# TorchIO-project/torchio

Hardware: AMD Instinct MI355X
Metric: volumes/s (256^3 float32) for Compose[affine+elastic+bias+blur+noise] (higher is better)
Workload: dtype f32; 1 GPU; Compose[Affine(+-10deg,0.9-1.1,+-5mm),ElasticDeformation(7^3cp,7.5mm),BiasField,Blur(0.5-2mm),Noise] on 1x256^3 f32, per-instance params; batch_per_gpu=8, global_batch=8, noise_rng=philox, resample_precision=tight, stencil_precision=fast, parallelism=batch-split x1 (no data-path collective)

## Files before the change

torchio_amd/csrc/stencil_march.hpp:

```cpp
#pragma once

#include "common.hpp"
#include "philox_normal.hpp"

namespace tio {

constexpr int kBlock = 256;

struct ConvArgs {
  const void* src;
  void* dst;
  const void* x_orig;
  const float* taps;
  const uint8_t* skip;
  int I, J, K;
  int channels;
  int axis, radius;
  int taps_batched, tap_stride;
  int orig_dtype;
  int last_pass;
  int tiles_a;
  int bcs;
  int radius_k;
  const float* bias_coarse;
  int bias_ci, bias_cj, bias_ck;
  float bias_si, bias_sj, bias_sk;
  int noise_on, noise_batched;
  float noise_mean, noise_std;
  const float* noise_mean_b;
  const float* noise_std_b;
  uint64_t noise_seed;
  const float* noise_base;
  int fma;
};

constexpr int kMarchMaxRadius = 8;
#ifndef TIO_MARCH_AHEAD
#define TIO_MARCH_AHEAD 2
#endif
constexpr int kMarchAhead = TIO_MARCH_AHEAD;

template <int R, bool FUSE_K, bool PRE_BIAS, int POST_NOISE, bool FMA>
__global__ __launch_bounds__(kBlock, (FUSE_K && !PRE_BIAS && R <= 6) ? 4 : 1) void conv_march_kernel(const ConvArgs a) {
  constexpr int W = 2 * R + 1;
  typedef float v4f __attribute__((ext_vector_type(4)));
  typedef __attribute__((address_space(4))) const float* const_float_ptr;
  extern __shared__ __attribute__((aligned(16))) float s_mem[];
  const int lane = threadIdx.x & 63, wave = __builtin_amdgcn_readfirstlane(threadIdx.x >> 6);
  float* s_krow = s_mem + wave * 272;
  (void)s_krow;
  const int n_other = a.axis == 0 ? a.J : a.I;
  const int strip_block = a.tiles_a ? blockIdx.x : blockIdx.z;
  const int k_tile = a.tiles_a ? blockIdx.z : blockIdx.x;
  const int strip = strip_block * (kBlock / 64) + wave;
  if (strip >= n_other * a.bcs) return;
  const int other = strip % n_other;
  const int bc = strip / n_other;
  const int b = bc / a.channels;
  const int k = k_tile * 256 + 4 * lane;
  const int n = a.axis == 0 ? a.I : a.J;
  const int seg = (n + gridDim.y - 1) / gridDim.y;
  const int p_begin = blockIdx.y * seg, p_end = min(p_begin + seg, n);
  const int64_t n_spatial = static_cast<int64_t>(a.I) * a.J * a.K;
  const int64_t stride = a.axis == 0 ? static_cast<int64_t>(a.J) * a.K : a.K;
  const int64_t other_stride = a.axis == 0 ? a.K : static_cast<int64_t>(a.J) * a.K;
  const int64_t line = static_cast<int64_t>(bc) * n_spatial + other * other_stride + k;
  const float* src = static_cast<const float*>(a.src);
  float* dst = static_cast<float*>(a.dst);
  if (p_begin >= p_end || k >= a.K) return;

  if (a.skip != nullptr && a.skip[b] != 0) {
    if (a.last_pass) {
      const float* orig = static_cast<const float*>(a.x_orig);
      for (int p = p_begin; p < p_end; p++) {
        const int64_t e = line + static_cast<int64_t>(p) * stride;
        *reinterpret_cast<v4f*>(dst + e) = *reinterpret_cast<const v4f*>(orig + e);
      }
    }
    return;
  }
  const int64_t tap_base = a.taps_batched ? static_cast<int64_t>(b) * 3 * a.tap_stride : 0;
  const_float_ptr tc = (const_float_ptr)(a.taps + tap_base + static_cast<int64_t>(a.axis) * a.tap_stride);
  const_float_ptr tk = (const_float_ptr)(a.taps + tap_base + 2 * a.tap_stride);
  (void)tk;
  float tw[W];
#pragma unroll
  for (int t = 0; t < W; t++) tw[t] = tc[t];
  float tkw[17];
  (void)tkw;
  if constexpr (FUSE_K) {
    const int rk0 = a.radius_k;
#pragma unroll
    for (int jj = 0; jj < 17; jj++) {
      const int t = jj - (8 - rk0);
      tkw[jj] = (t >= 0 && t <= 2 * rk0) ? tk[t] : 0.0f;
    }
  }
  float noise_mu = a.noise_mean, noise_sd = a.noise_std;
  if constexpr (POST_NOISE != 0) {
    if (a.noise_batched) {
      noise_mu = ((const_float_ptr)a.noise_mean_b)[b];
      noise_sd = ((const_float_ptr)a.noise_std_b)[b];
    }
  }

  Lerp1D b_lk[4];
  Lerp1D b_lj{0, 0, 1.0f, 0.0f};
  float b_p0[4] = {0.f, 0.f, 0.f, 0.f}, b_p1[4] = {0.f, 0.f, 0.f, 0.f};
  int b_cur0 = -1, b_cur1 = -1;
  const float* b_fg = nullptr;
  if constexpr (PRE_BIAS) {
    b_fg = a.bias_coarse + static_cast<int64_t>(bc) * (a.bias_ci * a.bias_cj * a.bias_ck);
    b_lj = lerp_index(other, a.bias_cj, a.J, a.bias_sj);
#pragma unroll
    for (int e = 0; e < 4; e++) b_lk[e] = lerp_index(min(k + e, a.K - 1), a.bias_ck, a.K, a.bias_sk);
  }
  auto bias_row = [&](v4f v, int pos) -> v4f {
    if constexpr (PRE_BIAS) {
      const Lerp1D li = lerp_index(pos, a.bias_ci, a.I, a.bias_si);
      const int s_i = a.bias_cj * a.bias_ck, s_j = a.bias_ck;
      auto plane = [&](int ii, float (&out)[4]) {
        const float* r0 = b_fg + ii * s_i + b_lj.i0 * s_j;
        const float* r1 = b_fg + ii * s_i + b_lj.i1 * s_j;
#pragma unroll
        for (int e = 0; e < 4; e++)
          out[e] = lerp2(lerp2(r0[b_lk[e].i0], b_lk[e].l0, r0[b_lk[e].i1], b_lk[e].l1), b_lj.l0,
                         lerp2(r1[b_lk[e].i0], b_lk[e].l0, r1[b_lk[e].i1], b_lk[e].l1), b_lj.l1);
      };
      if (li.i0 != b_cur0) {
        if (li.i0 == b_cur1) {
#pragma unroll
          for (int e = 0; e < 4; e++) b_p0[e] = b_p1[e];
        } else {
          plane(li.i0, b_p0);
        }
        b_cur0 = li.i0;
      }
      if (li.i1 != b_cur1) {
        if (li.i1 == b_cur0) {
#pragma unroll
          for (int e = 0; e < 4; e++) b_p1[e] = b_p0[e];
        } else {
          plane(li.i1, b_p1);
        }
        b_cur1 = li.i1;
      }
      v.x = __fmul_rn(v.x, expf(lerp2(b_p0[0], li.l0, b_p1[0], li.l1)));
      v.y = __fmul_rn(v.y, expf(lerp2(b_p0[1], li.l0, b_p1[1], li.l1)));
      v.z = __fmul_rn(v.z, expf(lerp2(b_p0[2], li.l0, b_p1[2], li.l1)));
      v.w = __fmul_rn(v.w, expf(lerp2(b_p0[3], li.l0, b_p1[3], li.l1)));
    }
    return v;
  };
#define TIO_ROW_POS(P) min(max((P), 0), n - 1)
#define TIO_ROW_LOAD(P) (*reinterpret_cast<const v4f*>(src + line + static_cast<int64_t>(TIO_ROW_POS(P)) * stride))
  v4f win[W];
#pragma unroll
  for (int t = 0; t < 2 * R; t++) win[t] = bias_row(TIO_ROW_LOAD(p_begin - R + t), TIO_ROW_POS(p_begin - R + t));
  win[2 * R] = win[0];
  v4f nxt[kMarchAhead];
#pragma unroll
  for (int d = 0; d < kMarchAhead; d++) nxt[d] = TIO_ROW_LOAD(p_begin + R + d);
  for (int p0 = p_begin; p0 < p_end; p0 += W) {
#pragma unroll
    for (int u = 0; u < W; u++) {
      const int p = p0 + u;
      if (p >= p_end) return;
      __builtin_amdgcn_sched_barrier(0);
      win[(2 * R + u) % W] = bias_row(nxt[0], TIO_ROW_POS(p + R));
#pragma unroll
      for (int d = 0; d + 1 < kMarchAhead; d++) nxt[d] = nxt[d + 1];
      v4f zrow = {0.0f, 0.0f, 0.0f, 0.0f};
      if constexpr (POST_NOISE == 2) zrow = __builtin_nontemporal_load(reinterpret_cast<const v4f*>(a.noise_base + line + static_cast<int64_t>(p) * stride));
      (void)zrow;
      nxt[kMarchAhead - 1] = TIO_ROW_LOAD(p + R + kMarchAhead);
      float4 acc = make_float4(0.0f, 0.0f, 0.0f, 0.0f);
      if constexpr (FMA) {
#pragma unroll
        for (int t = 0; t < W; t++) {
          const v4f v = win[(u + t) % W];
          acc.x = __builtin_fmaf(tw[t], v.x, acc.x);
          acc.y = __builtin_fmaf(tw[t], v.y, acc.y);
          acc.z = __builtin_fmaf(tw[t], v.z, acc.z);
          acc.w = __builtin_fmaf(tw[t], v.w, acc.w);
        }
      } else {
#pragma unroll
        for (int t = 0; t < W; t++) {
          const v4f v = win[(u + t) % W];
          acc.x = __fadd_rn(acc.x, __fmul_rn(tw[t], v.x));
          acc.y = __fadd_rn(acc.y, __fmul_rn(tw[t], v.y));
          acc.z = __fadd_rn(acc.z, __fmul_rn(tw[t], v.z));
          acc.w = __fadd_rn(acc.w, __fmul_rn(tw[t], v.w));
        }
      }
      if constexpr (FUSE_K) {
        int rk = a.radius_k;
        if constexpr (!FMA) asm volatile("" : "+s"(rk));
        const float edge_l = __int_as_float(__builtin_amdgcn_readlane(__float_as_int(acc.x), 0));
        const float edge_r = __int_as_float(__builtin_amdgcn_readlane(__float_as_int(acc.w), a.K / 4 - 1));
        *reinterpret_cast<float4*>(s_krow + 8 + 4 * lane) = acc;
        for (int h = lane; h < 16; h += a.K / 4) {
          if (h < 8) s_krow[h] = edge_l;
          else s_krow[8 + a.K + (h - 8)] = edge_r;
        }
        __builtin_amdgcn_fence(__ATOMIC_ACQ_REL, "wavefront");
        __builtin_amdgcn_wave_barrier();
        const float4* rv = reinterpret_cast<const float4*>(s_krow + 8) + lane;
        float w[20];
#pragma unroll
        for (int d = 0; d < 5; d++) {
          const float4 c = rv[d - 2];
          w[4 * d] = c.x; w[4 * d + 1] = c.y; w[4 * d + 2] = c.z; w[4 * d + 3] = c.w;
        }
        float4 out = make_float4(0.0f, 0.0f, 0.0f, 0.0f);
        if constexpr (FMA) {
#define TIO_K_TIER(T)                                              \
  _Pragma("unroll") for (int jj = 8 - (T); jj <= 8 + (T); jj++) { \
    const float tv = tkw[jj];                                      \
    out.x = __builtin_fmaf(tv, w[jj], out.x);                      \
    out.y = __builtin_fmaf(tv, w[jj + 1], out.y);                  \
    out.z = __builtin_fmaf(tv, w[jj + 2], out.z);                  \
    out.w = __builtin_fmaf(tv, w[jj + 3], out.w);                  \
  }
          if (rk <= 4) { TIO_K_TIER(4) } else if (rk <= 6) { TIO_K_TIER(6) } else { TIO_K_TIER(8) }
#undef TIO_K_TIER
        } else {
#define TIO_K_TAP(JJ)                                       \
  {                                                         \
    const float tv = tkw[JJ];                               \
    out.x = __fadd_rn(out.x, __fmul_rn(tv, w[(JJ)]));       \
    out.y = __fadd_rn(out.y, __fmul_rn(tv, w[(JJ) + 1]));   \
    out.z = __fadd_rn(out.z, __fmul_rn(tv, w[(JJ) + 2]));   \
    out.w = __fadd_rn(out.w, __fmul_rn(tv, w[(JJ) + 3]));   \
  }
          if (rk <= 4) {
#pragma unroll
            for (int jj = 4; jj <= 12; jj++) {
              if (jj >= 7 && jj <= 9) TIO_K_TAP(jj)
              else if (jj >= 8 - rk && jj <= 8 + rk) TIO_K_TAP(jj)
            }
          } else if (rk <= 6) {
            if (rk == 6) TIO_K_TAP(2)
#pragma unroll
            for (int jj = 3; jj <= 13; jj++) TIO_K_TAP(jj)
            if (rk == 6) TIO_K_TAP(14)
          } else {
            if (rk == 8) TIO_K_TAP(0)
#pragma unroll
            for (int jj = 1; jj <= 15; jj++) TIO_K_TAP(jj)
            if (rk == 8) TIO_K_TAP(16)
          }
#undef TIO_K_TAP
        }
        acc = out;
        __builtin_amdgcn_fence(__ATOMIC_ACQ_REL, "wavefront");
        __builtin_amdgcn_wave_barrier();
        if constexpr (POST_NOISE != 0) {
          const int64_t e0 = line + static_cast<int64_t>(p) * stride;
          float z[4];
          if constexpr (POST_NOISE == 2) {
            z[0] = zrow.x; z[1] = zrow.y; z[2] = zrow.z; z[3] = zrow.w;
          } else {
            philox_normal4(a.noise_seed, 0, static_cast<uint64_t>(e0 >> 2), z);
          }
          const float mu = noise_mu, sd = noise_sd;
          acc.x = __fadd_rn(acc.x, __fadd_rn(mu, __fmul_rn(sd, z[0])));
          acc.y = __fadd_rn(acc.y, __fadd_rn(mu, __fmul_rn(sd, z[1])));
          acc.z = __fadd_rn(acc.z, __fadd_rn(mu, __fmul_rn(sd, z[2])));
          acc.w = __fadd_rn(acc.w, __fadd_rn(mu, __fmul_rn(sd, z[3])));
        }
      }
      *reinterpret_cast<float4*>(dst + line + static_cast<int64_t>(p) * stride) = acc;
    }
  }
#undef TIO_ROW_LOAD
#undef TIO_ROW_POS
}

void launch_conv_march_fused(int radius_class, int post_noise, bool fma, dim3 grid, size_t lds, hipStream_t stream, const ConvArgs& a);

}
```

Measured before the change: 6120 volumes/s.

## Specialize fused blur march kernel on runtime effective tap radius

The march body moves into an include file and is instantiated once per effective radius from 1 to R for the FMA fused-K path. At runtime each wave counts the symmetric zero outer taps in both the marching and the K filters, then dispatches to a body with a narrower register window and fewer FMAs, taking the K tier from the trimmed radius. Per-instance blur sigmas pad the tap arrays with zeros, so skipping those taps removes wasted loads and FMAs. The cost is more code size and instruction cache pressure, possible register changes from several inlined bodies, and a per-wave branch.

```diff
diff --git a/torchio_amd/csrc/stencil_march.hpp b/torchio_amd/csrc/stencil_march.hpp
--- a/torchio_amd/csrc/stencil_march.hpp
+++ b/torchio_amd/csrc/stencil_march.hpp
@@ -39,6 +39,7 @@
 #define TIO_MARCH_AHEAD 2
 #endif
 constexpr int kMarchAhead = TIO_MARCH_AHEAD;
+constexpr int kMarchOwnRadiusMax = 6;
 
 template <int R, bool FUSE_K, bool PRE_BIAS, int POST_NOISE, bool FMA>
 __global__ __launch_bounds__(kBlock, (FUSE_K && !PRE_BIAS && R <= 6) ? 4 : 1) void conv_march_kernel(const ConvArgs a) {
@@ -104,178 +105,70 @@
     }
   }
 
-  Lerp1D b_lk[4];
-  Lerp1D b_lj{0, 0, 1.0f, 0.0f};
-  float b_p0[4] = {0.f, 0.f, 0.f, 0.f}, b_p1[4] = {0.f, 0.f, 0.f, 0.f};
-  int b_cur0 = -1, b_cur1 = -1;
-  const float* b_fg = nullptr;
-  if constexpr (PRE_BIAS) {
-    b_fg = a.bias_coarse + static_cast<int64_t>(bc) * (a.bias_ci * a.bias_cj * a.bias_ck);
-    b_lj = lerp_index(other, a.bias_cj, a.J, a.bias_sj);
+  if constexpr (FMA && FUSE_K && !PRE_BIAS && R <= kMarchOwnRadiusMax) {
+    int lead = 0, lead_k = 0;
+    bool outer_zero = true;
 #pragma unroll
-    for (int e = 0; e < 4; e++) b_lk[e] = lerp_index(min(k + e, a.K - 1), a.bias_ck, a.K, a.bias_sk);
+    for (int t = 0; t < R - 1; t++) {
+      outer_zero = outer_zero && ((__float_as_int(tw[t]) | __float_as_int(tw[2 * R - t])) << 1) == 0;
+      lead += outer_zero ? 1 : 0;
+    }
+    outer_zero = true;
+#pragma unroll
+    for (int jj = 0; jj < 7; jj++) {
+      outer_zero = outer_zero && ((__float_as_int(tkw[jj]) | __float_as_int(tkw[16 - jj])) << 1) == 0;
+      lead_k += outer_zero ? 1 : 0;
+    }
+    const int r_own = R - lead;
+    int rk_tier = 8 - lead_k;
+    asm volatile("" : "+v"(rk_tier), "+v"(noise_mu), "+v"(noise_sd));
+    if (r_own == 1) {
+      constexpr int RB = 1, WB = 2 * RB + 1, tap_first = R - RB;
+#include "stencil_march_body.inc"
+      return;
+    }
+    if constexpr (R >= 2) {
+      if (r_own == 2) {
+        constexpr int RB = 2, WB = 2 * RB + 1, tap_first = R - RB;
+#include "stencil_march_body.inc"
+        return;
+      }
+    }
+    if constexpr (R >= 3) {
+      if (r_own == 3) {
+        constexpr int RB = 3, WB = 2 * RB + 1, tap_first = R - RB;
+#include "stencil_march_body.inc"
+        return;
+      }
+    }
+    if constexpr (R >= 4) {
+      if (r_own == 4) {
+        constexpr int RB = 4, WB = 2 * RB + 1, tap_first = R - RB;
+#include "stencil_march_body.inc"
+        return;
+      }
+    }
+    if constexpr (R >= 5) {
+      if (r_own == 5) {
+        constexpr int RB = 5, WB = 2 * RB + 1, tap_first = R - RB;
+#include "stencil_march_body.inc"
+        return;
+      }
+    }
+    if constexpr (R >= 6) {
+      if (r_own == 6) {
+        constexpr int RB = 6, WB = 2 * RB + 1, tap_first = R - RB;
+#include "stencil_march_body.inc"
+        return;
+      }
+    }
+    static_assert(kMarchOwnRadiusMax == 6, "one case per radius up to kMarchOwnRadiusMax");
+  } else {
+    constexpr int RB = R, WB = W, tap_first = 0;
+    const int rk_tier = a.radius_k;
+    (void)rk_tier;
+#include "stencil_march_body.inc"
   }
-  auto bias_row = [&](v4f v, int pos) -> v4f {
-    if constexpr (PRE_BIAS) {
-      const Lerp1D li = lerp_index(pos, a.bias_ci, a.I, a.bias_si);
-      const int s_i = a.bias_cj * a.bias_ck, s_j = a.bias_ck;
-      auto plane = [&](int ii, float (&out)[4]) {
-        const float* r0 = b_fg + ii * s_i + b_lj.i0 * s_j;
-        const float* r1 = b_fg + ii * s_i + b_lj.i1 * s_j;
-#pragma unroll
-        for (int e = 0; e < 4; e++)
-          out[e] = lerp2(lerp2(r0[b_lk[e].i0], b_lk[e].l0, r0[b_lk[e].i1], b_lk[e].l1), b_lj.l0,
-                         lerp2(r1[b_lk[e].i0], b_lk[e].l0, r1[b_lk[e].i1], b_lk[e].l1), b_lj.l1);
-      };
-      if (li.i0 != b_cur0) {
-        if (li.i0 == b_cur1) {
-#pragma unroll
-          for (int e = 0; e < 4; e++) b_p0[e] = b_p1[e];
-        } else {
-          plane(li.i0, b_p0);
-        }
-        b_cur0 = li.i0;
-      }
-      if (li.i1 != b_cur1) {
-        if (li.i1 == b_cur0) {
-#pragma unroll
-          for (int e = 0; e < 4; e++) b_p1[e] = b_p0[e];
-        } else {
-          plane(li.i1, b_p1);
-        }
-        b_cur1 = li.i1;
-      }
-      v.x = __fmul_rn(v.x, expf(lerp2(b_p0[0], li.l0, b_p1[0], li.l1)));
-      v.y = __fmul_rn(v.y, expf(lerp2(b_p0[1], li.l0, b_p1[1], li.l1)));
-      v.z = __fmul_rn(v.z, expf(lerp2(b_p0[2], li.l0, b_p1[2], li.l1)));
-      v.w = __fmul_rn(v.w, expf(lerp2(b_p0[3], li.l0, b_p1[3], li.l1)));
-    }
-    return v;
-  };
-#define TIO_ROW_POS(P) min(max((P), 0), n - 1)
-#define TIO_ROW_LOAD(P) (*reinterpret_cast<const v4f*>(src + line + static_cast<int64_t>(TIO_ROW_POS(P)) * stride))
-  v4f win[W];
-#pragma unroll
-  for (int t = 0; t < 2 * R; t++) win[t] = bias_row(TIO_ROW_LOAD(p_begin - R + t), TIO_ROW_POS(p_begin - R + t));
-  win[2 * R] = win[0];
-  v4f nxt[kMarchAhead];
-#pragma unroll
-  for (int d = 0; d < kMarchAhead; d++) nxt[d] = TIO_ROW_LOAD(p_begin + R + d);
-  for (int p0 = p_begin; p0 < p_end; p0 += W) {
-#pragma unroll
-    for (int u = 0; u < W; u++) {
-      const int p = p0 + u;
-      if (p >= p_end) return;
-      __builtin_amdgcn_sched_barrier(0);
-      win[(2 * R + u) % W] = bias_row(nxt[0], TIO_ROW_POS(p + R));
-#pragma unroll
-      for (int d = 0; d + 1 < kMarchAhead; d++) nxt[d] = nxt[d + 1];
-      v4f zrow = {0.0f, 0.0f, 0.0f, 0.0f};
-      if constexpr (POST_NOISE == 2) zrow = __builtin_nontemporal_load(reinterpret_cast<const v4f*>(a.noise_base + line + static_cast<int64_t>(p) * stride));
-      (void)zrow;
-      nxt[kMarchAhead - 1] = TIO_ROW_LOAD(p + R + kMarchAhead);
-      float4 acc = make_float4(0.0f, 0.0f, 0.0f, 0.0f);
-      if constexpr (FMA) {
-#pragma unroll
-        for (int t = 0; t < W; t++) {
-          const v4f v = win[(u + t) % W];
-          acc.x = __builtin_fmaf(tw[t], v.x, acc.x);
-          acc.y = __builtin_fmaf(tw[t], v.y, acc.y);
-          acc.z = __builtin_fmaf(tw[t], v.z, acc.z);
-          acc.w = __builtin_fmaf(tw[t], v.w, acc.w);
-        }
-      } else {
-#pragma unroll
-        for (int t = 0; t < W; t++) {
-          const v4f v = win[(u + t) % W];
-          acc.x = __fadd_rn(acc.x, __fmul_rn(tw[t], v.x));
-          acc.y = __fadd_rn(acc.y, __fmul_rn(tw[t], v.y));
-          acc.z = __fadd_rn(acc.z, __fmul_rn(tw[t], v.z));
-          acc.w = __fadd_rn(acc.w, __fmul_rn(tw[t], v.w));
-        }
-      }
-      if constexpr (FUSE_K) {
-        int rk = a.radius_k;
-        if constexpr (!FMA) asm volatile("" : "+s"(rk));
-        const float edge_l = __int_as_float(__builtin_amdgcn_readlane(__float_as_int(acc.x), 0));
-        const float edge_r = __int_as_float(__builtin_amdgcn_readlane(__float_as_int(acc.w), a.K / 4 - 1));
-        *reinterpret_cast<float4*>(s_krow + 8 + 4 * lane) = acc;
-        for (int h = lane; h < 16; h += a.K / 4) {
-          if (h < 8) s_krow[h] = edge_l;
-          else s_krow[8 + a.K + (h - 8)] = edge_r;
-        }
-        __builtin_amdgcn_fence(__ATOMIC_ACQ_REL, "wavefront");
-        __builtin_amdgcn_wave_barrier();
-        const float4* rv = reinterpret_cast<const float4*>(s_krow + 8) + lane;
-        float w[20];
-#pragma unroll
-        for (int d = 0; d < 5; d++) {
-          const float4 c = rv[d - 2];
-          w[4 * d] = c.x; w[4 * d + 1] = c.y; w[4 * d + 2] = c.z; w[4 * d + 3] = c.w;
-        }
-        float4 out = make_float4(0.0f, 0.0f, 0.0f, 0.0f);
-        if constexpr (FMA) {
-#define TIO_K_TIER(T)                                              \
-  _Pragma("unroll") for (int jj = 8 - (T); jj <= 8 + (T); jj++) { \
-    const float tv = tkw[jj];                                      \
-    out.x = __builtin_fmaf(tv, w[jj], out.x);                      \
-    out.y = __builtin_fmaf(tv, w[jj + 1], out.y);                  \
-    out.z = __builtin_fmaf(tv, w[jj + 2], out.z);                  \
-    out.w = __builtin_fmaf(tv, w[jj + 3], out.w);                  \
-  }
-          if (rk <= 4) { TIO_K_TIER(4) } else if (rk <= 6) { TIO_K_TIER(6) } else { TIO_K_TIER(8) }
-#undef TIO_K_TIER
-        } else {
-#define TIO_K_TAP(JJ)                                       \
-  {                                                         \
-    const float tv = tkw[JJ];                               \
-    out.x = __fadd_rn(out.x, __fmul_rn(tv, w[(JJ)]));       \
-    out.y = __fadd_rn(out.y, __fmul_rn(tv, w[(JJ) + 1]));   \
-    out.z = __fadd_rn(out.z, __fmul_rn(tv, w[(JJ) + 2]));   \
-    out.w = __fadd_rn(out.w, __fmul_rn(tv, w[(JJ) + 3]));   \
-  }
-          if (rk <= 4) {
-#pragma unroll
-            for (int jj = 4; jj <= 12; jj++) {
-              if (jj >= 7 && jj <= 9) TIO_K_TAP(jj)
-              else if (jj >= 8 - rk && jj <= 8 + rk) TIO_K_TAP(jj)
-            }
-          } else if (rk <= 6) {
-            if (rk == 6) TIO_K_TAP(2)
-#pragma unroll
-            for (int jj = 3; jj <= 13; jj++) TIO_K_TAP(jj)
-            if (rk == 6) TIO_K_TAP(14)
-          } else {
-            if (rk == 8) TIO_K_TAP(0)
-#pragma unroll
-            for (int jj = 1; jj <= 15; jj++) TIO_K_TAP(jj)
-            if (rk == 8) TIO_K_TAP(16)
-          }
-#undef TIO_K_TAP
-        }
-        acc = out;
-        __builtin_amdgcn_fence(__ATOMIC_ACQ_REL, "wavefront");
-        __builtin_amdgcn_wave_barrier();
-        if constexpr (POST_NOISE != 0) {
-          const int64_t e0 = line + static_cast<int64_t>(p) * stride;
-          float z[4];
-          if constexpr (POST_NOISE == 2) {
-            z[0] = zrow.x; z[1] = zrow.y; z[2] = zrow.z; z[3] = zrow.w;
-          } else {
-            philox_normal4(a.noise_seed, 0, static_cast<uint64_t>(e0 >> 2), z);
-          }
-          const float mu = noise_mu, sd = noise_sd;
-          acc.x = __fadd_rn(acc.x, __fadd_rn(mu, __fmul_rn(sd, z[0])));
-          acc.y = __fadd_rn(acc.y, __fadd_rn(mu, __fmul_rn(sd, z[1])));
-          acc.z = __fadd_rn(acc.z, __fadd_rn(mu, __fmul_rn(sd, z[2])));
-          acc.w = __fadd_rn(acc.w, __fadd_rn(mu, __fmul_rn(sd, z[3])));
-        }
-      }
-      *reinterpret_cast<float4*>(dst + line + static_cast<int64_t>(p) * stride) = acc;
-    }
-  }
-#undef TIO_ROW_LOAD
-#undef TIO_ROW_POS
 }
 
 void launch_conv_march_fused(int radius_class, int post_noise, bool fma, dim3 grid, size_t lds, hipStream_t stream, const ConvArgs& a);
diff --git a/torchio_amd/csrc/stencil_march_body.inc b/torchio_amd/csrc/stencil_march_body.inc
--- /dev/null
+++ b/torchio_amd/csrc/stencil_march_body.inc
@@ -0,0 +1,172 @@
+  Lerp1D b_lk[4];
+  Lerp1D b_lj{0, 0, 1.0f, 0.0f};
+  float b_p0[4] = {0.f, 0.f, 0.f, 0.f}, b_p1[4] = {0.f, 0.f, 0.f, 0.f};
+  int b_cur0 = -1, b_cur1 = -1;
+  const float* b_fg = nullptr;
+  if constexpr (PRE_BIAS) {
+    b_fg = a.bias_coarse + static_cast<int64_t>(bc) * (a.bias_ci * a.bias_cj * a.bias_ck);
+    b_lj = lerp_index(other, a.bias_cj, a.J, a.bias_sj);
+#pragma unroll
+    for (int e = 0; e < 4; e++) b_lk[e] = lerp_index(min(k + e, a.K - 1), a.bias_ck, a.K, a.bias_sk);
+  }
+  auto bias_row = [&](v4f v, int pos) -> v4f {
+    if constexpr (PRE_BIAS) {
+      const Lerp1D li = lerp_index(pos, a.bias_ci, a.I, a.bias_si);
+      const int s_i = a.bias_cj * a.bias_ck, s_j = a.bias_ck;
+      auto plane = [&](int ii, float (&out)[4]) {
+        const float* r0 = b_fg + ii * s_i + b_lj.i0 * s_j;
+        const float* r1 = b_fg + ii * s_i + b_lj.i1 * s_j;
+#pragma unroll
+        for (int e = 0; e < 4; e++)
+          out[e] = lerp2(lerp2(r0[b_lk[e].i0], b_lk[e].l0, r0[b_lk[e].i1], b_lk[e].l1), b_lj.l0,
+                         lerp2(r1[b_lk[e].i0], b_lk[e].l0, r1[b_lk[e].i1], b_lk[e].l1), b_lj.l1);
+      };
+      if (li.i0 != b_cur0) {
+        if (li.i0 == b_cur1) {
+#pragma unroll
+          for (int e = 0; e < 4; e++) b_p0[e] = b_p1[e];
+        } else {
+          plane(li.i0, b_p0);
+        }
+        b_cur0 = li.i0;
+      }
+      if (li.i1 != b_cur1) {
+        if (li.i1 == b_cur0) {
+#pragma unroll
+          for (int e = 0; e < 4; e++) b_p1[e] = b_p0[e];
+        } else {
+          plane(li.i1, b_p1);
+        }
+        b_cur1 = li.i1;
+      }
+      v.x = __fmul_rn(v.x, expf(lerp2(b_p0[0], li.l0, b_p1[0], li.l1)));
+      v.y = __fmul_rn(v.y, expf(lerp2(b_p0[1], li.l0, b_p1[1], li.l1)));
+      v.z = __fmul_rn(v.z, expf(lerp2(b_p0[2], li.l0, b_p1[2], li.l1)));
+      v.w = __fmul_rn(v.w, expf(lerp2(b_p0[3], li.l0, b_p1[3], li.l1)));
+    }
+    return v;
+  };
+#define TIO_ROW_POS(P) min(max((P), 0), n - 1)
+#define TIO_ROW_LOAD(P) (*reinterpret_cast<const v4f*>(src + line + static_cast<int64_t>(TIO_ROW_POS(P)) * stride))
+  v4f win[WB];
+#pragma unroll
+  for (int t = 0; t < 2 * RB; t++) win[t] = bias_row(TIO_ROW_LOAD(p_begin - RB + t), TIO_ROW_POS(p_begin - RB + t));
+  win[2 * RB] = win[0];
+  v4f nxt[kMarchAhead];
+#pragma unroll
+  for (int d = 0; d < kMarchAhead; d++) nxt[d] = TIO_ROW_LOAD(p_begin + RB + d);
+  for (int p0 = p_begin; p0 < p_end; p0 += WB) {
+#pragma unroll
+    for (int u = 0; u < WB; u++) {
+      const int p = p0 + u;
+      if (p >= p_end) return;
+      __builtin_amdgcn_sched_barrier(0);
+      win[(2 * RB + u) % WB] = bias_row(nxt[0], TIO_ROW_POS(p + RB));
+#pragma unroll
+      for (int d = 0; d + 1 < kMarchAhead; d++) nxt[d] = nxt[d + 1];
+      v4f zrow = {0.0f, 0.0f, 0.0f, 0.0f};
+      if constexpr (POST_NOISE == 2) zrow = __builtin_nontemporal_load(reinterpret_cast<const v4f*>(a.noise_base + line + static_cast<int64_t>(p) * stride));
+      (void)zrow;
+      nxt[kMarchAhead - 1] = TIO_ROW_LOAD(p + RB + kMarchAhead);
+      float4 acc = make_float4(0.0f, 0.0f, 0.0f, 0.0f);
+      if constexpr (FMA) {
+#pragma unroll
+        for (int t = 0; t < WB; t++) {
+          const v4f v = win[(u + t) % WB];
+          acc.x = __builtin_fmaf(tw[tap_first + t], v.x, acc.x);
+          acc.y = __builtin_fmaf(tw[tap_first + t], v.y, acc.y);
+          acc.z = __builtin_fmaf(tw[tap_first + t], v.z, acc.z);
+          acc.w = __builtin_fmaf(tw[tap_first + t], v.w, acc.w);
+        }
+      } else {
+#pragma unroll
+        for (int t = 0; t < WB; t++) {
+          const v4f v = win[(u + t) % WB];
+          acc.x = __fadd_rn(acc.x, __fmul_rn(tw[tap_first + t], v.x));
+          acc.y = __fadd_rn(acc.y, __fmul_rn(tw[tap_first + t], v.y));
+          acc.z = __fadd_rn(acc.z, __fmul_rn(tw[tap_first + t], v.z));
+          acc.w = __fadd_rn(acc.w, __fmul_rn(tw[tap_first + t], v.w));
+        }
+      }
+      if constexpr (FUSE_K) {
+        int rk = rk_tier;
+        if constexpr (!FMA) asm volatile("" : "+s"(rk));
+        const float edge_l = __int_as_float(__builtin_amdgcn_readlane(__float_as_int(acc.x), 0));
+        const float edge_r = __int_as_float(__builtin_amdgcn_readlane(__float_as_int(acc.w), a.K / 4 - 1));
+        *reinterpret_cast<float4*>(s_krow + 8 + 4 * lane) = acc;
+        for (int h = lane; h < 16; h += a.K / 4) {
+          if (h < 8) s_krow[h] = edge_l;
+          else s_krow[8 + a.K + (h - 8)] = edge_r;
+        }
+        __builtin_amdgcn_fence(__ATOMIC_ACQ_REL, "wavefront");
+        __builtin_amdgcn_wave_barrier();
+        const float4* rv = reinterpret_cast<const float4*>(s_krow + 8) + lane;
+        float w[20];
+#pragma unroll
+        for (int d = 0; d < 5; d++) {
+          const float4 c = rv[d - 2];
+          w[4 * d] = c.x; w[4 * d + 1] = c.y; w[4 * d + 2] = c.z; w[4 * d + 3] = c.w;
+        }
+        float4 out = make_float4(0.0f, 0.0f, 0.0f, 0.0f);
+        if constexpr (FMA) {
+#define TIO_K_TIER(T)                                              \
+  _Pragma("unroll") for (int jj = 8 - (T); jj <= 8 + (T); jj++) { \
+    const float tv = tkw[jj];                                      \
+    out.x = __builtin_fmaf(tv, w[jj], out.x);                      \
+    out.y = __builtin_fmaf(tv, w[jj + 1], out.y);                  \
+    out.z = __builtin_fmaf(tv, w[jj + 2], out.z);                  \
+    out.w = __builtin_fmaf(tv, w[jj + 3], out.w);                  \
+  }
+          if (rk <= 4) { TIO_K_TIER(4) } else if (rk <= 6) { TIO_K_TIER(6) } else { TIO_K_TIER(8) }
+#undef TIO_K_TIER
+        } else {
+#define TIO_K_TAP(JJ)                                       \
+  {                                                         \
+    const float tv = tkw[JJ];                               \
+    out.x = __fadd_rn(out.x, __fmul_rn(tv, w[(JJ)]));       \
+    out.y = __fadd_rn(out.y, __fmul_rn(tv, w[(JJ) + 1]));   \
+    out.z = __fadd_rn(out.z, __fmul_rn(tv, w[(JJ) + 2]));   \
+    out.w = __fadd_rn(out.w, __fmul_rn(tv, w[(JJ) + 3]));   \
+  }
+          if (rk <= 4) {
+#pragma unroll
+            for (int jj = 4; jj <= 12; jj++) {
+              if (jj >= 7 && jj <= 9) TIO_K_TAP(jj)
+              else if (jj >= 8 - rk && jj <= 8 + rk) TIO_K_TAP(jj)
+            }
+          } else if (rk <= 6) {
+            if (rk == 6) TIO_K_TAP(2)
+#pragma unroll
+            for (int jj = 3; jj <= 13; jj++) TIO_K_TAP(jj)
+            if (rk == 6) TIO_K_TAP(14)
+          } else {
+            if (rk == 8) TIO_K_TAP(0)
+#pragma unroll
+            for (int jj = 1; jj <= 15; jj++) TIO_K_TAP(jj)
+            if (rk == 8) TIO_K_TAP(16)
+          }
+#undef TIO_K_TAP
+        }
+        acc = out;
+        __builtin_amdgcn_fence(__ATOMIC_ACQ_REL, "wavefront");
+        __builtin_amdgcn_wave_barrier();
+        if constexpr (POST_NOISE != 0) {
+          const int64_t e0 = line + static_cast<int64_t>(p) * stride;
+          float z[4];
+          if constexpr (POST_NOISE == 2) {
+            z[0] = zrow.x; z[1] = zrow.y; z[2] = zrow.z; z[3] = zrow.w;
+          } else {
+            philox_normal4(a.noise_seed, 0, static_cast<uint64_t>(e0 >> 2), z);
+          }
+          const float mu = noise_mu, sd = noise_sd;
+          acc.x = __fadd_rn(acc.x, __fadd_rn(mu, __fmul_rn(sd, z[0])));
+          acc.y = __fadd_rn(acc.y, __fadd_rn(mu, __fmul_rn(sd, z[1])));
+          acc.z = __fadd_rn(acc.z, __fadd_rn(mu, __fmul_rn(sd, z[2])));
+          acc.w = __fadd_rn(acc.w, __fadd_rn(mu, __fmul_rn(sd, z[3])));
+        }
+      }
+      *reinterpret_cast<float4*>(dst + line + static_cast<int64_t>(p) * stride) = acc;
+    }
+  }
+#undef TIO_ROW_LOAD
+#undef TIO_ROW_POS
```

Result: no change. 6126 volumes/s, median of 2 (+0.1%).
